# zeromq/libzmq

Hardware: AMD Instinct MI355X
Metric: GiB/s device-resident CURVE encode+decode, 1 KiB-msg batches; msgs/s (higher is better)
Workload: dtype u32; 1 GPU; config2: 65536 x 1024 B frames, 1 CURVE session per GPU, encode+decode round trip; frames_per_gpu=65536, payload_bytes=1024, wire_bytes=1057, sessions=1, parallelism=frame-sharded x1, no collective

## Files before the change

### libzmq_amd/csrc/curve_device.hpp

```cpp
#pragma once

#include <hip/hip_runtime.h>
#include <stdint.h>

namespace zmqg {

__device__ __forceinline__ uint32_t rotl32(uint32_t x, uint32_t n)
{
    return __builtin_rotateleft32(x, n);
}

#define ZMQG_QR(a, b, c, d)        \
    b ^= rotl32(a + d, 7);         \
    c ^= rotl32(b + a, 9);         \
    d ^= rotl32(c + b, 13);        \
    a ^= rotl32(d + c, 18);

#define ZMQG_SALSA20_ROUNDS(x)                                   \
    _Pragma("unroll") for (int rr_ = 0; rr_ < 10; ++rr_)         \
    {                                                            \
        ZMQG_QR(x[0], x[4], x[8], x[12]);                        \
        ZMQG_QR(x[5], x[9], x[13], x[1]);                        \
        ZMQG_QR(x[10], x[14], x[2], x[6]);                       \
        ZMQG_QR(x[15], x[3], x[7], x[11]);                       \
        ZMQG_QR(x[0], x[1], x[2], x[3]);                         \
        ZMQG_QR(x[5], x[6], x[7], x[4]);                         \
        ZMQG_QR(x[10], x[11], x[8], x[9]);                       \
        ZMQG_QR(x[15], x[12], x[13], x[14]);                     \
    }

constexpr uint32_t SIGMA0 = 0x61707865, SIGMA1 = 0x3320646e, SIGMA2 = 0x79622d32, SIGMA3 = 0x6b206574;

__device__ __forceinline__ void salsa20_block(uint32_t out[16], const uint32_t k[8], uint32_t n0, uint32_t n1,
                                              uint32_t ctr_lo, uint32_t ctr_hi)
{
    uint32_t x[16] = {SIGMA0, k[0], k[1], k[2], k[3], SIGMA1, n0, n1,
                      ctr_lo, ctr_hi, SIGMA2, k[4], k[5], k[6], k[7], SIGMA3};
    ZMQG_SALSA20_ROUNDS(x);
    out[0] = x[0] + SIGMA0;
    out[1] = x[1] + k[0];
    out[2] = x[2] + k[1];
    out[3] = x[3] + k[2];
    out[4] = x[4] + k[3];
    out[5] = x[5] + SIGMA1;
    out[6] = x[6] + n0;
    out[7] = x[7] + n1;
    out[8] = x[8] + ctr_lo;
    out[9] = x[9] + ctr_hi;
    out[10] = x[10] + SIGMA2;
    out[11] = x[11] + k[4];
    out[12] = x[12] + k[5];
    out[13] = x[13] + k[6];
    out[14] = x[14] + k[7];
    out[15] = x[15] + SIGMA3;
}

__device__ __forceinline__ void hsalsa20(uint32_t out[8], const uint32_t k[8], const uint32_t in[4])
{
    uint32_t x[16] = {SIGMA0, k[0], k[1], k[2], k[3], SIGMA1, in[0], in[1],
                      in[2], in[3], SIGMA2, k[4], k[5], k[6], k[7], SIGMA3};
    ZMQG_SALSA20_ROUNDS(x);
    out[0] = x[0];
    out[1] = x[5];
    out[2] = x[10];
    out[3] = x[15];
    out[4] = x[6];
    out[5] = x[7];
    out[6] = x[8];
    out[7] = x[9];
}

constexpr uint32_t M26 = 0x3ffffff;

struct fe {
    uint32_t l[5];
};

__device__ __forceinline__ fe fe_zero()
{
    fe z;
    z.l[0] = z.l[1] = z.l[2] = z.l[3] = z.l[4] = 0;
    return z;
}

__device__ __forceinline__ fe fe_one()
{
    fe o = fe_zero();
    o.l[0] = 1;
    return o;
}

__device__ __forceinline__ fe poly_r_from_key(uint32_t k0, uint32_t k1, uint32_t k2, uint32_t k3)
{
    fe r;
    r.l[0] = k0 & 0x3ffffff;
    r.l[1] = __builtin_amdgcn_alignbit(k1, k0, 26) & 0x3ffff03;
    r.l[2] = __builtin_amdgcn_alignbit(k2, k1, 20) & 0x3ffc0ff;
    r.l[3] = __builtin_amdgcn_alignbit(k3, k2, 14) & 0x3f03fff;
    r.l[4] = (k3 >> 8) & 0x00fffff;
    return r;
}

__device__ __forceinline__ void fe_add_block(fe &h, uint32_t m0, uint32_t m1, uint32_t m2, uint32_t m3,
                                             uint32_t hibit)
{
    h.l[0] += m0 & M26;
    h.l[1] += __builtin_amdgcn_alignbit(m1, m0, 26) & M26;
    h.l[2] += __builtin_amdgcn_alignbit(m2, m1, 20) & M26;
    h.l[3] += __builtin_amdgcn_alignbit(m3, m2, 14) & M26;
    h.l[4] += (m3 >> 8) | hibit;
}

__device__ __forceinline__ void fe_add(fe &h, const fe &x)
{
#pragma unroll
    for (int i = 0; i < 5; ++i)
        h.l[i] += x.l[i];
}

__device__ __forceinline__ uint64_t mad64(uint32_t a, uint32_t b, uint64_t c)
{
    return (uint64_t) a * b + c;
}

__device__ __forceinline__ void fe_mul_s(fe &h, const fe &r, const uint32_t s1, const uint32_t s2, const uint32_t s3,
                                         const uint32_t s4)
{
    const uint32_t h0 = h.l[0], h1 = h.l[1], h2 = h.l[2], h3 = h.l[3], h4 = h.l[4];
    uint64_t d0 = mad64(h4, s1, mad64(h3, s2, mad64(h2, s3, mad64(h1, s4, (uint64_t) h0 * r.l[0]))));
    uint64_t d1 = mad64(h4, s2, mad64(h3, s3, mad64(h2, s4, mad64(h1, r.l[0], (uint64_t) h0 * r.l[1]))));
    uint64_t d2 = mad64(h4, s3, mad64(h3, s4, mad64(h2, r.l[0], mad64(h1, r.l[1], (uint64_t) h0 * r.l[2]))));
    uint64_t d3 = mad64(h4, s4, mad64(h3, r.l[0], mad64(h2, r.l[1], mad64(h1, r.l[2], (uint64_t) h0 * r.l[3]))));
    uint64_t d4 = mad64(h4, r.l[0], mad64(h3, r.l[1], mad64(h2, r.l[2], mad64(h1, r.l[3], (uint64_t) h0 * r.l[4]))));
    uint32_t c;
    c = (uint32_t) (d0 >> 26);
    h.l[0] = (uint32_t) d0 & M26;
    d1 += c;
    c = (uint32_t) (d1 >> 26);
    h.l[1] = (uint32_t) d1 & M26;
    d2 += c;
    c = (uint32_t) (d2 >> 26);
    h.l[2] = (uint32_t) d2 & M26;
    d3 += c;
    c = (uint32_t) (d3 >> 26);
    h.l[3] = (uint32_t) d3 & M26;
    d4 += c;
    c = (uint32_t) (d4 >> 26);
    h.l[4] = (uint32_t) d4 & M26;
    h.l[0] += c * 5;
    c = h.l[0] >> 26;
    h.l[0] &= M26;
    h.l[1] += c;
}

__device__ __forceinline__ void fe_mul(fe &h, const fe &r)
{
    fe_mul_s(h, r, r.l[1] * 5, r.l[2] * 5, r.l[3] * 5, r.l[4] * 5);
}

__device__ __forceinline__ fe fe_from_wide(const uint64_t w[5])
{
    uint64_t a0 = w[0], a1 = w[1], a2 = w[2], a3 = w[3], a4 = w[4];
    a1 += a0 >> 26;
    a0 &= M26;
    a2 += a1 >> 26;
    a1 &= M26;
    a3 += a2 >> 26;
    a2 &= M26;
    a4 += a3 >> 26;
    a3 &= M26;
    a0 += (a4 >> 26) * 5;
    a4 &= M26;
    a1 += a0 >> 26;
    a0 &= M26;
    fe h;
    h.l[0] = (uint32_t) a0;
    h.l[1] = (uint32_t) a1;
    h.l[2] = (uint32_t) a2;
    h.l[3] = (uint32_t) a3;
    h.l[4] = (uint32_t) a4;
    return h;
}

__device__ __forceinline__ void poly_finish(fe h, const uint32_t s[4], uint32_t tag[4])
{
    uint32_t h0 = h.l[0], h1 = h.l[1], h2 = h.l[2], h3 = h.l[3], h4 = h.l[4], c;
    c = h1 >> 26;
    h1 &= M26;
    h2 += c;
    c = h2 >> 26;
    h2 &= M26;
    h3 += c;
    c = h3 >> 26;
    h3 &= M26;
    h4 += c;
    c = h4 >> 26;
    h4 &= M26;
    h0 += c * 5;
    c = h0 >> 26;
    h0 &= M26;
    h1 += c;
    uint32_t g0 = h0 + 5;
    c = g0 >> 26;
    g0 &= M26;
    uint32_t g1 = h1 + c;
    c = g1 >> 26;
    g1 &= M26;
    uint32_t g2 = h2 + c;
    c = g2 >> 26;
    g2 &= M26;
    uint32_t g3 = h3 + c;
    c = g3 >> 26;
    g3 &= M26;
    uint32_t g4 = h4 + c - (1u << 26);
    const uint32_t mask = (g4 >> 31) - 1u;
    h0 = (h0 & ~mask) | (g0 & mask);
    h1 = (h1 & ~mask) | (g1 & mask);
    h2 = (h2 & ~mask) | (g2 & mask);
    h3 = (h3 & ~mask) | (g3 & mask);
    h4 = (h4 & ~mask) | (g4 & mask);
    uint64_t f0 = (uint64_t) (h0 | (h1 << 26)) + s[0];
    uint64_t f1 = (uint64_t) ((h1 >> 6) | (h2 << 20)) + s[1] + (f0 >> 32);
    uint64_t f2 = (uint64_t) ((h2 >> 12) | (h3 << 14)) + s[2] + (f1 >> 32);
    uint64_t f3 = (uint64_t) ((h3 >> 18) | (h4 << 8)) + s[3] + (f2 >> 32);
    tag[0] = (uint32_t) f0;
    tag[1] = (uint32_t) f1;
    tag[2] = (uint32_t) f2;
    tag[3] = (uint32_t) f3;
}

__device__ __forceinline__ void poly_absorb64(fe &h, const fe &r, const uint32_t s1, const uint32_t s2,
                                              const uint32_t s3, const uint32_t s4, uint32_t w[16], int nv)
{
    if (nv >= 64) {
#pragma unroll
        for (int q = 0; q < 4; ++q) {
            fe_add_block(h, w[4 * q], w[4 * q + 1], w[4 * q + 2], w[4 * q + 3], 1u << 24);
            fe_mul_s(h, r, s1, s2, s3, s4);
        }
        return;
    }
#pragma unroll
    for (int q = 0; q < 4; ++q) {
        const int bl = nv - 16 * q;
        if (bl <= 0)
            break;
        uint32_t m[4] = {w[4 * q], w[4 * q + 1], w[4 * q + 2], w[4 * q + 3]};
        uint32_t hibit = 1u << 24;
        if (bl < 16) {
            hibit = 0;
            const int wi = bl >> 2, bi = bl & 3;
#pragma unroll
            for (int t = 0; t < 4; ++t)
                if (t == wi)
                    m[t] |= 1u << (8 * bi);
        }
        fe_add_block(h, m[0], m[1], m[2], m[3], hibit);
        fe_mul_s(h, r, s1, s2, s3, s4);
    }
}

struct Poly32 {
    uint32_t h0, h1, h2, h3, h4;
};

struct PolyKey32 {
    uint32_t r0, r1, r2, r3, s1, s2, s3;
};

__device__ __forceinline__ PolyKey32 poly32_key(uint32_t k0, uint32_t k1, uint32_t k2, uint32_t k3)
{
    PolyKey32 k;
    k.r0 = k0 & 0x0fffffffu;
    k.r1 = k1 & 0x0ffffffcu;
    k.r2 = k2 & 0x0ffffffcu;
    k.r3 = k3 & 0x0ffffffcu;
    k.s1 = k.r1 + (k.r1 >> 2);
    k.s2 = k.r2 + (k.r2 >> 2);
    k.s3 = k.r3 + (k.r3 >> 2);
    return k;
}

__device__ __forceinline__ void poly32_block(Poly32 &h, uint32_t m0, uint32_t m1, uint32_t m2, uint32_t m3,
                                             uint32_t hib, const PolyKey32 &k)
{
    unsigned c;
    const uint32_t a0 = __builtin_addc(h.h0, m0, 0u, &c);
    const uint32_t a1 = __builtin_addc(h.h1, m1, c, &c);
    const uint32_t a2 = __builtin_addc(h.h2, m2, c, &c);
    const uint32_t a3 = __builtin_addc(h.h3, m3, c, &c);
    const uint32_t a4 = h.h4 + hib + c;
    const uint64_t d0 = mad64(a3, k.s1, mad64(a2, k.s2, mad64(a1, k.s3, (uint64_t) a0 * k.r0)));
    const uint64_t d1 = mad64(a4, k.s1, mad64(a3, k.s2, mad64(a2, k.s3, mad64(a1, k.r0, (uint64_t) a0 * k.r1))));
    const uint64_t d2 = mad64(a4, k.s2, mad64(a3, k.s3, mad64(a2, k.r0, mad64(a1, k.r1, (uint64_t) a0 * k.r2))));
    const uint64_t d3 = mad64(a4, k.s3, mad64(a3, k.r0, mad64(a2, k.r1, mad64(a1, k.r2, (uint64_t) a0 * k.r3))));
    const uint32_t h0 = (uint32_t) d0;
    const uint32_t h1 = __builtin_addc((uint32_t) d1, (uint32_t) (d0 >> 32), 0u, &c);
    const uint32_t c1 = (uint32_t) (d1 >> 32) + c;
    const uint32_t h2 = __builtin_addc((uint32_t) d2, c1, 0u, &c);
    const uint32_t c2 = (uint32_t) (d2 >> 32) + c;
    const uint32_t h3 = __builtin_addc((uint32_t) d3, c2, 0u, &c);
    const uint32_t h4 = a4 * k.r0 + (uint32_t) (d3 >> 32) + c;
    const uint32_t f = (h4 >> 2) + (h4 & ~3u);
    h.h0 = __builtin_addc(h0, f, 0u, &c);
    h.h1 = __builtin_addc(h1, 0u, c, &c);
    h.h2 = __builtin_addc(h2, 0u, c, &c);
    h.h3 = __builtin_addc(h3, 0u, c, &c);
    h.h4 = (h4 & 3u) + c;
}

__device__ __forceinline__ void poly32_window(Poly32 &h, const PolyKey32 &k, const uint32_t c[16], uint32_t j0,
                                              uint32_t len)
{
#pragma unroll
    for (int j = 0; j < 4; ++j) {
        const int off = 16 * (j - (int) j0);
        if (j >= (int) j0 && off < (int) len) {
            const int nb = (int) len - off;
            uint32_t m0 = c[4 * j], m1 = c[4 * j + 1], m2 = c[4 * j + 2], m3 = c[4 * j + 3], hib = 1u;
            if (nb < 16) {
                hib = 0u;
                const uint32_t pad = 1u << (8 * (nb & 3));
                const int wi = nb >> 2;
                m0 |= wi == 0 ? pad : 0u;
                m1 |= wi == 1 ? pad : 0u;
                m2 |= wi == 2 ? pad : 0u;
                m3 |= wi == 3 ? pad : 0u;
            }
            poly32_block(h, m0, m1, m2, m3, hib, k);
        }
    }
}

__device__ __forceinline__ void poly32_window_full(Poly32 &h, const PolyKey32 &k, const uint32_t c[16])
{
#pragma unroll
    for (int j = 0; j < 4; ++j)
        poly32_block(h, c[4 * j], c[4 * j + 1], c[4 * j + 2], c[4 * j + 3], 1u, k);
}

__device__ __forceinline__ PolyKey32 poly32_key_from_fe(const uint32_t r[5])
{
    return poly32_key(r[0] | (r[1] << 26), (r[1] >> 6) | (r[2] << 20), (r[2] >> 12) | (r[3] << 14),
                      (r[3] >> 18) | (r[4] << 8));
}

__device__ __forceinline__ Poly32 fe_to_poly32(fe x)
{
    uint32_t c;
    c = x.l[0] >> 26;
    x.l[0] &= M26;
    x.l[1] += c;
    c = x.l[1] >> 26;
    x.l[1] &= M26;
    x.l[2] += c;
    c = x.l[2] >> 26;
    x.l[2] &= M26;
    x.l[3] += c;
    c = x.l[3] >> 26;
    x.l[3] &= M26;
    x.l[4] += c;
    Poly32 h;
    h.h0 = x.l[0] | (x.l[1] << 26);
    h.h1 = (x.l[1] >> 6) | (x.l[2] << 20);
    h.h2 = (x.l[2] >> 12) | (x.l[3] << 14);
    h.h3 = (x.l[3] >> 18) | (x.l[4] << 8);
    h.h4 = x.l[4] >> 24;
    return h;
}

__device__ __forceinline__ fe poly32_to_fe(const Poly32 &h)
{
    fe x;
    x.l[0] = h.h0 & M26;
    x.l[1] = ((h.h0 >> 26) | (h.h1 << 6)) & M26;
    x.l[2] = ((h.h1 >> 20) | (h.h2 << 12)) & M26;
    x.l[3] = ((h.h2 >> 14) | (h.h3 << 18)) & M26;
    x.l[4] = (h.h3 >> 8) | (h.h4 << 24);
    return x;
}

__device__ __forceinline__ void poly32_finish(const Poly32 &h, const uint32_t s[4], uint32_t tag[4])
{
    unsigned c;
    const uint32_t g0 = __builtin_addc(h.h0, 5u, 0u, &c);
    const uint32_t g1 = __builtin_addc(h.h1, 0u, c, &c);
    const uint32_t g2 = __builtin_addc(h.h2, 0u, c, &c);
    const uint32_t g3 = __builtin_addc(h.h3, 0u, c, &c);
    const uint32_t g4 = h.h4 + c;
    const uint32_t m = 0u - (g4 >> 2);
    const uint32_t f0 = (g0 & m) | (h.h0 & ~m), f1 = (g1 & m) | (h.h1 & ~m), f2 = (g2 & m) | (h.h2 & ~m),
                   f3 = (g3 & m) | (h.h3 & ~m);
    tag[0] = __builtin_addc(f0, s[0], 0u, &c);
    tag[1] = __builtin_addc(f1, s[1], c, &c);
    tag[2] = __builtin_addc(f2, s[2], c, &c);
    tag[3] = __builtin_addc(f3, s[3], c, &c);
}

__device__ __forceinline__ uint32_t bswap32(uint32_t x)
{
    return __builtin_bswap32(x);
}

__device__ __forceinline__ void mask_tail(uint32_t w[16], int nv)
{
#pragma unroll
    for (int i = 0; i < 16; ++i) {
        const int b = nv - 4 * i;
        const uint32_t m = b >= 4 ? 0xffffffffu : (b <= 0 ? 0u : ((1u << (8 * b)) - 1u));
        w[i] &= m;
    }
}

__device__ __forceinline__ void load_window(const uint8_t *p, int nv, uint32_t w[16])
{
    const uint32_t sh = (uint32_t) ((uintptr_t) p & 3);
    const uint32_t *q = (const uint32_t *) (p - sh);
    uint32_t d[17];
    if (nv >= 64) {
#pragma unroll
        for (int i = 0; i < 16; ++i)
            d[i] = q[i];
        d[16] = sh ? q[16] : 0u;
    } else {
        const int nd = (int) ((sh + (uint32_t) nv + 3) >> 2);
#pragma unroll
        for (int i = 0; i < 17; ++i)
            d[i] = i < nd ? q[i] : 0u;
    }
#pragma unroll
    for (int i = 0; i < 16; ++i)
        w[i] = __builtin_amdgcn_alignbyte(d[i + 1], d[i], sh);
    if (nv < 64)
        mask_tail(w, nv);
}

__device__ __forceinline__ void store_window(uint8_t *p, int nv, const uint32_t w[16])
{
    const uintptr_t a = (uintptr_t) p;
    const uint32_t sh = (uint32_t) (a & 3);
    if (sh == 0 && nv >= 64) {
        typedef unsigned int u32x4_ __attribute__((ext_vector_type(4)));
        typedef __attribute__((address_space(1))) u32x4_ __attribute__((aligned(4))) GU4a4_;
#pragma unroll
        for (int i = 0; i < 4; ++i)
            *(GU4a4_ *) (a + 16u * i) = (u32x4_){w[4 * i], w[4 * i + 1], w[4 * i + 2], w[4 * i + 3]};
        return;
    }
    const uint32_t s = (4u - sh) & 3u;
    (void) a;
    uint32_t e[16];
#pragma unroll
    for (int k = 0; k < 15; ++k)
        e[k] = __builtin_amdgcn_alignbyte(w[k + 1], w[k], s);
    e[15] = __builtin_amdgcn_alignbyte(0u, w[15], s);
    const int lead = (int) s < nv ? (int) s : nv;
#pragma unroll
    for (int b = 0; b < 3; ++b)
        if (b < lead)
            p[b] = (uint8_t) (w[0] >> (8 * b));
    if (nv <= (int) s)
        return;
    const int rem = nv - (int) s;
    const int nd = rem >> 2;
    uint32_t *q = (uint32_t *) (p + s);
#pragma unroll
    for (int k = 0; k < 16; ++k)
        if (k < nd)
            q[k] = e[k];
    const int tb = rem & 3;
    if (tb) {
        uint32_t t = 0;
#pragma unroll
        for (int k = 0; k < 16; ++k)
            if (k == nd)
                t = e[k];
        uint8_t *pt = (uint8_t *) (q + nd);
#pragma unroll
        for (int b = 0; b < 3; ++b)
            if (b < tb)
                pt[b] = (uint8_t) (t >> (8 * b));
    }
}

template <int NV>
__device__ __forceinline__ void store_bytes_c(uint8_t *p, const uint32_t w[16])
{
    static_assert(NV % 4 == 0 && NV >= 8 && NV <= 64, "whole dwords, at most one window");
    typedef __attribute__((address_space(1))) uint8_t GU8_;
    typedef __attribute__((address_space(1))) uint16_t GU16_;
    typedef __attribute__((address_space(1))) uint32_t GU32_;
    typedef unsigned int u32x2_ __attribute__((ext_vector_type(2)));
    typedef unsigned int u32x3_ __attribute__((ext_vector_type(3)));
    typedef __attribute__((address_space(1))) u32x2_ __attribute__((aligned(4))) GU2a4_;
    typedef __attribute__((address_space(1))) u32x3_ __attribute__((aligned(4))) GU3a4_;
    typedef unsigned int u32x4_ __attribute__((ext_vector_type(4)));
    typedef __attribute__((address_space(1))) u32x4_ __attribute__((aligned(4))) GU4a4_;
    const uint64_t a = (uint64_t) (uintptr_t) p;
    const uint32_t sh = (uint32_t) a & 3u, s = (4u - sh) & 3u;
    constexpr int ND = NV / 4;
    uint32_t e[ND];
#pragma unroll
    for (int k = 0; k < ND; ++k)
        e[k] = __builtin_amdgcn_alignbyte(k + 1 < 16 ? w[k + 1] : 0u, w[k], s);
    if (s & 1u)
        *(GU8_ *) (uintptr_t) a = (uint8_t) w[0];
    if (s & 2u)
        *(GU16_ *) (uintptr_t) (a + (s & 1u)) = (uint16_t) (w[0] >> (8u * (s & 1u)));
    const uint64_t q = a + s;
    constexpr int NU = ND - 1;
#pragma unroll
    for (int g = 0; g + 4 <= NU; g += 4)
        *(GU4a4_ *) (uintptr_t) (q + 4u * g) = (u32x4_){e[g], e[g + 1], e[g + 2], e[g + 3]};
    constexpr int G4 = NU / 4 * 4;
    if (NU - G4 == 3)
        *(GU3a4_ *) (uintptr_t) (q + 4u * G4) = (u32x3_){e[G4], e[G4 + 1], e[G4 + 2]};
    else if (NU - G4 == 2)
        *(GU2a4_ *) (uintptr_t) (q + 4u * G4) = (u32x2_){e[G4], e[G4 + 1]};
    else if (NU - G4 == 1)
        *(GU32_ *) (uintptr_t) (q + 4u * G4) = e[G4];
    if (s == 0u)
        *(GU32_ *) (uintptr_t) (q + 4u * NU) = e[NU];
    const uint64_t t = q + 4u * NU;
    if (sh & 2u)
        *(GU16_ *) (uintptr_t) t = (uint16_t) e[NU];
    if (sh & 1u)
        *(GU8_ *) (uintptr_t) (t + (sh & 2u)) = (uint8_t) (e[NU] >> (8u * (sh & 2u)));
}

template <int NV>
__device__ __forceinline__ void load_bytes_c(const uint8_t *p, uint32_t w[NV / 4])
{
    static_assert(NV % 16 == 0 && NV >= 16 && NV <= 48, "whole granules");
    typedef __attribute__((address_space(1))) const uint32_t GCU32_;
    typedef unsigned int u32x4_ __attribute__((ext_vector_type(4)));
    typedef __attribute__((address_space(1))) const u32x4_ __attribute__((aligned(4))) GCU4a4_;
    const uint64_t a = (uint64_t) (uintptr_t) p;
    const uint32_t sh = (uint32_t) a & 3u;
    const uint64_t q = a - sh;
    constexpr int ND = NV / 4;
    uint32_t d[ND + 1];
#pragma unroll
    for (int g = 0; g < ND / 4; ++g) {
        const u32x4_ t = *(GCU4a4_ *) (uintptr_t) (q + 16u * g);
        d[4 * g] = t.x;
        d[4 * g + 1] = t.y;
        d[4 * g + 2] = t.z;
        d[4 * g + 3] = t.w;
    }
    d[ND] = sh ? *(GCU32_ *) (uintptr_t) (q + 4u * ND) : 0u;
#pragma unroll
    for (int k = 0; k < ND; ++k)
        w[k] = __builtin_amdgcn_alignbyte(d[k + 1], d[k], sh);
}

__device__ __forceinline__ void store_tail(uint64_t a, uint32_t nb, const uint32_t o[17])
{
    typedef __attribute__((address_space(1))) uint8_t GU8_;
    typedef __attribute__((address_space(1))) uint16_t GU16_;
    typedef __attribute__((address_space(1))) uint32_t GU32_;
    typedef unsigned int u32x4_ __attribute__((ext_vector_type(4)));
    typedef __attribute__((address_space(1))) u32x4_ __attribute__((aligned(4))) GU4a4_;
    const uint32_t nw = nb >> 2, ng = nw >> 2;
#pragma unroll
    for (uint32_t g = 0; g < 4; ++g)
        if (g < ng)
            *(GU4a4_ *) (uintptr_t) (a + 16u * g) = (u32x4_){o[4 * g], o[4 * g + 1], o[4 * g + 2], o[4 * g + 3]};
    uint32_t r[4];
#pragma unroll
    for (uint32_t k = 0; k < 4; ++k) {
        uint32_t v = 0;
#pragma unroll
        for (uint32_t g = 0; g < 5; ++g)
            if (g == ng && 4 * g + k < 17)
                v = o[4 * g + k];
        r[k] = v;
    }
    const uint64_t b = a + 16u * ng;
    const uint32_t nr = nw - 4u * ng;
#pragma unroll
    for (uint32_t k = 0; k < 3; ++k)
        if (k < nr)
            *(GU32_ *) (uintptr_t) (b + 4u * k) = r[k];
    uint32_t last = r[0];
#pragma unroll
    for (uint32_t k = 1; k < 4; ++k)
        if (k == nr)
            last = r[k];
    const uint32_t tb = nb & 3u;
    const uint64_t c = b + 4u * nr;
    if (tb & 2u)
        *(GU16_ *) (uintptr_t) c = (uint16_t) last;
    if (tb & 1u)
        *(GU8_ *) (uintptr_t) (c + (tb & 2u)) = (uint8_t) (last >> (8u * (tb & 2u)));
}

__device__ __forceinline__ void zero_bytes(uint8_t *p, uint32_t len)
{
    const uint32_t head = (uint32_t) ((16u - ((uintptr_t) p & 15u)) & 15u);
    const uint32_t h = head < len ? head : len;
    for (uint32_t b = 0; b < h; ++b)
        p[b] = 0;
    uint32_t k = h;
    typedef unsigned int z4 __attribute__((ext_vector_type(4)));
    for (; k + 16u <= len; k += 16u)
        *(z4 *) (p + k) = (z4){0u, 0u, 0u, 0u};
    for (; k < len; ++k)
        p[k] = 0;
}

typedef unsigned int u32x4 __attribute__((ext_vector_type(4)));
typedef __attribute__((address_space(1))) uint8_t GU8;
typedef __attribute__((address_space(1))) const u32x4 GCU4;
typedef __attribute__((address_space(1))) u32x4 GU4;
typedef __attribute__((address_space(1))) uint32_t GU32;

template <int N>
__device__ __forceinline__ void select_shift(const uint32_t *v, uint32_t ws, uint32_t *out)
{
    const uint32_t m1 = 0u - (ws & 1u), m2 = 0u - ((ws >> 1) & 1u);
    uint32_t a[N + 2];
#pragma unroll
    for (int i = 0; i < N + 2; ++i)
        a[i] = (v[i + 1] & m1) | (v[i] & ~m1);
#pragma unroll
    for (int i = 0; i < N; ++i)
        out[i] = (a[i + 2] & m2) | (a[i] & ~m2);
}

struct StreamReader {
    const GCU4 *g;
    uint32_t off;
    uint32_t end;
    u32x4 carry;
};

__device__ __forceinline__ void reader_init(StreamReader &r, uint64_t p, uint32_t L)
{
    r.off = (uint32_t) (p & 15);
    r.g = (const GCU4 *) (uintptr_t) (p - r.off);
    r.end = r.off + L;
// ... 155 lines not shown
```

### libzmq_amd/csrc/curve_frames.hpp

```cpp
#pragma once

#ifndef ZMQG_FRAMES_ABLATE
#define ZMQG_FRAMES_ABLATE 0
#endif


#ifndef ZMQG_SEQ_STORE
#define ZMQG_SEQ_STORE 0
#endif

__device__ __forceinline__ void seq_store4(uint64_t a, uint32_t x, uint32_t y, uint32_t z, uint32_t w)
{
    typedef unsigned int v4_ __attribute__((ext_vector_type(4)));
    typedef __attribute__((address_space(1))) v4_ __attribute__((aligned(4))) G4_;
    if (ZMQG_SEQ_STORE == 3)
        asm volatile("global_store_dwordx4 %0, %1, off sc0 sc1\n\ts_nop 1" ::"v"(a), "v"((v4_){x, y, z, w}) : "memory");
    else
        *(G4_ *) (uintptr_t) a = (v4_){x, y, z, w};
}

#ifndef ZMQG_SEQ_COOPST
#define ZMQG_SEQ_COOPST 2
#endif
#ifndef ZMQG_SEQ_SKIP5
// ... 1014 lines not shown
        sh_cs = c0;
    __syncthreads();
    const CallState cs = sh_cs;
    const uint32_t epoch = cs.epoch;
    const uint32_t wg = use_ticket ? cs.ticket : blockIdx.x;
    if (use_ticket)
        fetch(wg);
    const uint64_t nbase = cs.nbase;
    unsigned long long *const list_ctr = zs->list_ctr + (epoch & 1u);
    if (blockIdx.x == 0 && threadIdx.x == 0)
        zs->list_ctr[(epoch & 1u) ^ 1u] = 0;

    if (!DEC) {
        const uint64_t nc = frame_nonce(nonce, ctl, nbase, ii);
        n0 = bswap32((uint32_t) (nc >> 32));
        n1 = bswap32((uint32_t) nc);
    } else {
        if (L_in < 64u)
            mask_tail(x0, (int) L_in);
        const uint32_t b0 = x0[0] & 0xffu;
        if (L_in <= 1u || L_in <= b0)
            status = ZMQG_ERR_MALFORMED_UNSPECIFIED;
        else if (L_in < 8u || x0[0] != 0x53454d07u || x0[1] != 0x45474153u)
            status = ZMQG_ERR_UNEXPECTED_COMMAND;
        else if (L_in < 33u)
            status = ZMQG_ERR_MALFORMED_MESSAGE;
        if (!sid_ok)
            status = ZMQG_ERR_SESSION;
        if (over)
            status = ZMQG_ERR_BOUND;
        n0 = x0[2];
        n1 = x0[3];
        S = status == 0 ? L_in : 0u;
    }
    const bool small = valid && S <= max_stream;
    unsigned long long vn = 0, wexcl = 0, psn = 0, wagg = 0;
    if (DEC) {
        vn = valid && status == 0 ? (((unsigned long long) bswap32(n0) << 32) | bswap32(n1)) : 0ull;
        psn = rp.peer[s];
        if (valid && !lb) {
            rp.vout[i] = vn;
            rp.psnap[i] = psn;
            if (rp.iota)
                rp.iota[i] = i;
        }
        if (lb) {
            const unsigned long long sc = wave_scan_max_u64(vn);
            const unsigned long long up = wave_prev_u64(sc);
            if (lane == 63)
                sh_wmax[threadIdx.x >> 6] = sc;
            __syncthreads();
            const uint32_t wv = threadIdx.x >> 6;
            for (uint32_t k = 0; k < kFramesWaves; ++k) {
                if (k < wv)
                    wexcl = sh_wmax[k] > wexcl ? sh_wmax[k] : wexcl;
                wagg = sh_wmax[k] > wagg ? sh_wmax[k] : wagg;
            }
            if (lane > 0)
                wexcl = up > wexcl ? up : wexcl;
            if (threadIdx.x == 0) {
                if (use_rec) {
                    __hip_atomic_store(rp.lb_rec + 2u * wg, lbrec_pack(epoch, (uint32_t) wagg), __ATOMIC_RELAXED,
                                       __HIP_MEMORY_SCOPE_AGENT);
                    __hip_atomic_store(rp.lb_rec + 2u * wg + 1u, lbrec_pack(epoch, (uint32_t) (wagg >> 32)),
                                       __ATOMIC_RELAXED, __HIP_MEMORY_SCOPE_AGENT);
                } else {
                    lookback_publish(rp.lb_flag + wg, rp.lb_agg + wg, wagg, epoch, 1);
                }
            }
        }
    }
    const bool is_big = valid && !small && S > 0;
    if (!small)
        S = 0;
    const uint32_t nw = (S + 63u) >> 6;
    const uint32_t steps = __builtin_amdgcn_readfirstlane(wave_max_u32(nw));
    __shared__ __attribute__((aligned(16))) uint8_t sq_lds[kFramesWaves * 2 * 64 * kStIn];
    uint8_t *const sq_w = sq_lds + (threadIdx.x >> 6) * 2 * 64 * kStIn;
    const uint32_t sq_off = __builtin_amdgcn_readfirstlane((uint32_t) (uintptr_t) (StLdsVoid *) sq_w);
    const uint32_t sq_va = (uint32_t) A & 15u;
    uint64_t sq_la[5];
    uint32_t sq_rel[5], sq_lim[5];
    {
        const uint64_t Ab = A - sq_va;
        const uint32_t lm = S ? sq_va + S : 0u;
#pragma unroll
        for (uint32_t j = 0; j < 5; ++j) {
            const uint32_t idx = 64u * j + lane, f = idx / 5u, k = idx - 5u * f;
            sq_rel[j] = 16u * k;
            sq_la[j] = shfl_u64(Ab, f) + sq_rel[j];
            sq_lim[j] = (uint32_t) __shfl((int) lm, (int) f);
            const int fva = __shfl((int) sq_va, (int) f);
            if (ZMQG_SEQ_SKIP5 && k == 4u && fva == 0)
                sq_lim[j] = 0;
        }
    }
    auto sq_dma = [&](uint32_t t) {
        const uint32_t b = __builtin_amdgcn_readfirstlane(sq_off + (t & 1u) * 64u * kStIn);
#pragma unroll
        for (uint32_t j = 0; j < 5; ++j)
            if (64u * t + sq_rel[j] < sq_lim[j])
                lds_dma16(sq_la[j] + 64ull * t, b + 1024u * j);
    };
    const uint32_t min_nw = __builtin_amdgcn_readfirstlane(~wave_max_u32(~nw));
    uint64_t sq_m[5];
#pragma unroll
    for (uint32_t j = 0; j < 5; ++j)
        sq_m[j] = __builtin_amdgcn_ballot_w64(sq_lim[j] != 0u);
    auto sq_dma_uni = [&](uint32_t t) {
        const uint32_t b = __builtin_amdgcn_readfirstlane(sq_off + (t & 1u) * 64u * kStIn);
        uint64_t a[5];
#pragma unroll
        for (uint32_t j = 0; j < 5; ++j)
            a[j] = sq_la[j] + 64ull * t;
        unsigned keep;
        uint64_t ex;
        asm volatile("s_mov_b32 %0, m0\n\t"
                     "s_mov_b64 %1, exec\n\t"
                     "s_mov_b32 m0, %7\n\t"
                     "s_mov_b64 exec, %8\n\t"
                     "global_load_lds_dwordx4 %2, off\n\t"
                     "s_add_u32 m0, m0, 0x400\n\t"
                     "s_mov_b64 exec, %9\n\t"
                     "global_load_lds_dwordx4 %3, off\n\t"
                     "s_add_u32 m0, m0, 0x400\n\t"
                     "s_mov_b64 exec, %10\n\t"
                     "global_load_lds_dwordx4 %4, off\n\t"
                     "s_add_u32 m0, m0, 0x400\n\t"
                     "s_mov_b64 exec, %11\n\t"
                     "global_load_lds_dwordx4 %5, off\n\t"
                     "s_add_u32 m0, m0, 0x400\n\t"
                     "s_mov_b64 exec, %12\n\t"
                     "global_load_lds_dwordx4 %6, off\n\t"
                     "s_mov_b64 exec, %1\n\t"
                     "s_mov_b32 m0, %0"
                     : "=&s"(keep), "=&s"(ex)
                     : "v"(a[0]), "v"(a[1]), "v"(a[2]), "v"(a[3]), "v"(a[4]), "s"(b), "s"(sq_m[0]), "s"(sq_m[1]),
                       "s"(sq_m[2]), "s"(sq_m[3]), "s"(sq_m[4])
                     : "memory", "scc");
    };
    if (steps > 1u && !(ZMQG_FRAMES_ABLATE & 16))
        sq_dma(1u);

    const bool al64 = ZMQG_SEQ_AL64 && DEC && __builtin_amdgcn_ballot_w64(((uint32_t) (uintptr_t) dst & 63u) != 0u) == 0;
    uint32_t yp[16];
    bool cs_pend = false;
    constexpr uint32_t kStgPlane = 64u * 16u + 16u;
    __shared__ __attribute__((aligned(16))) uint8_t sq_stg[ZMQG_SEQ_COOPST && SO ? kFramesWaves * 4 * kStgPlane : 16];
    uint8_t *const stg = sq_stg + (ZMQG_SEQ_COOPST && SO ? (threadIdx.x >> 6) * 4u * kStgPlane : 0u);
    auto stg_put = [&](uint32_t k) { return stg + kStgPlane * k + 16u * lane; };
    auto stg_get = [&](uint32_t j) { return stg + kStgPlane * (lane & 3u) + 16u * (16u * j + (lane >> 2)); };
    uint64_t cs_dst[4];
    uint32_t cs_nw[4];
    const bool coop = ZMQG_SEQ_COOPST && SO && (DEC ? al64 : true);
    if (coop) {
        const uint64_t cbase = DEC ? (uint64_t) (uintptr_t) dst : B - (((uint32_t) B & 3u) ? ((uint32_t) B & 3u) : 4u);
#pragma unroll
        for (uint32_t j = 0; j < 4; ++j) {
            const uint32_t f = 16u * j + (lane >> 2);
            cs_dst[j] = shfl_u64(cbase, f) + 16u * (lane & 3u);
            cs_nw[j] = (uint32_t) __shfl((int) nw, (int) f);
        }
    }
    uint32_t ct0[8];

    SEQ_STAMP(1u);
    PolyKey32 pk;
    Poly32 h = {0, 0, 0, 0, 0};
    uint32_t spad[4], wtag[4] = {0, 0, 0, 0}, fl = 0;
    uint32_t cp[16];
    uint32_t cp_j0 = 2, cp_len = 0;
    uint32_t ycarry;
    {
        uint32_t ks[16];
        salsa20_block(ks, key, n0, n1, 0, 0);
        pk = poly32_key(ks[0], ks[1], ks[2], ks[3]);
#pragma unroll
        for (int k = 0; k < 4; ++k)
            spad[k] = ks[4 + k];
        uint32_t x[16];
        if (DEC) {
#pragma unroll
            for (int k = 0; k < 16; ++k)
                x[k] = x0[k];
#pragma unroll
            for (int k = 0; k < 4; ++k)
                wtag[k] = x[4 + k];
        } else {
            uint32_t pt[8];
            switch (hl) {
            case 1: shift_in<1>(x0, pt); break;
            case 2: shift_in<2>(x0, pt); break;
            case 8: shift_in<8>(x0, pt); break;
            default: shift_in<11>(x0, pt); break;
            }
            pt[0] |= hw[0];
            pt[1] |= hw[1];
            pt[2] |= hw[2];
#pragma unroll
            for (int k = 0; k < 8; ++k) {
                x[k] = 0;
                x[8 + k] = pt[k];
            }
        }
        uint32_t y[16];
#pragma unroll
        for (int k = 0; k < 16; ++k)
            y[k] = x[k] ^ ks[k];
        if (!DEC && S < 64u)
            mask_tail(y, (int) S);
#pragma unroll
        for (int k = 0; k < 16; ++k)
            cp[k] = DEC ? x[k] : y[k];
        cp_len = (S < 64u ? S : 64u) - 32u;
        ycarry = y[15];
#pragma unroll
        for (int k = 0; k < 16; ++k)
            yp[k] = y[k];
        if (nw > 0) {
            if (DEC) {
                fl = y[8] & 3u;
                uint32_t pay[16];
#pragma unroll
                for (int k = 0; k < 7; ++k)
                    pay[k] = __builtin_amdgcn_alignbyte(y[9 + k], y[8 + k], 1);
                pay[7] = __builtin_amdgcn_alignbyte(0u, y[15], 1);
#pragma unroll
                for (int k = 8; k < 16; ++k)
                    pay[k] = 0;
                if (!al64 || nw == 1u)
                    store_window(dst, (int) (S < 64u ? S : 64u) - 33, pay);
            } else {
#pragma unroll
                for (int k = 0; k < 8; ++k)
                    ct0[k] = y[8 + k];
                if (S < 64u) {
                    uint32_t o[16];
                    o[0] = 0x53454d07u;
                    o[1] = 0x45474153u;
                    o[2] = n0;
                    o[3] = n1;
#pragma unroll
                    for (int k = 4; k < 16; ++k)
                        o[k] = 0;
                    store_bytes_c<16>(dst, o);
                    uint32_t ct[16];
#pragma unroll
                    for (int k = 0; k < 16; ++k)
                        ct[k] = k < 8 ? y[8 + k] : 0u;
                    store_window(dst + 32, (int) S - 32, ct);
                }
            }
        }
    }
    SEQ_STAMP(2u);
    call_state_count(zs);

    auto step = [&](auto uni, uint32_t t) {
        constexpr bool UNI = decltype(uni)::value;
        SEQ_STAMP(3u + t);
        const bool act = UNI || t < nw;
        const bool had = ZMQG_SEQ_COOPST && coop && cs_pend;
        u32x4 cg[4];
        if (had) {
            __builtin_amdgcn_fence(__ATOMIC_SEQ_CST, "wavefront");
#pragma unroll
            for (uint32_t j = 0; j < 4; ++j)
                cg[j] = *(const u32x4 *) stg_get(j);
        }
        uint32_t ks[16];
        if (ZMQG_FRAMES_ABLATE & 32) {
#pragma unroll
            for (int k = 0; k < 16; ++k)
                ks[k] = key[k & 7] ^ (t * 0x9e3779b9u + k);
        } else {
            salsa20_block(ks, key, n0, n1, t, 0);
        }
#pragma unroll
        for (int k = 0; k < 16; ++k)
            asm volatile("" : "+v"(ks[k]));
        SEQ_STAMP(24u + t);
        asm volatile("s_waitcnt vmcnt(0)" ::: "memory");
        __builtin_amdgcn_fence(__ATOMIC_SEQ_CST, "wavefront");
        uint32_t x[16];
        {
            const uint8_t *const p = sq_w + (t & 1u) * 64u * kStIn + kStIn * lane + sq_va;
#pragma unroll
            for (uint32_t q = 0; q < 4; ++q) {
                const u32x4 u = *(const u32x4_u1 *) (p + 16u * q);
                x[4 * q] = u.x;
                x[4 * q + 1] = u.y;
                x[4 * q + 2] = u.z;
                x[4 * q + 3] = u.w;
            }
        }
        asm volatile("" : "+v"(h.h0), "+v"(h.h1), "+v"(h.h2), "+v"(h.h3), "+v"(h.h4));
        const bool pv = UNI || t - 1u < nw;
        const bool full = UNI || (pv && cp_j0 == 0u && cp_len == 64u);
        {
            Poly32 hf = h;
            if (ZMQG_FRAMES_ABLATE & 64)
                hf.h0 ^= cp[0] ^ cp[5] ^ cp[11];
            else
                poly32_window_full(hf, pk, cp);
            h.h0 = full ? hf.h0 : h.h0;
            h.h1 = full ? hf.h1 : h.h1;
            h.h2 = full ? hf.h2 : h.h2;
            h.h3 = full ? hf.h3 : h.h3;
            h.h4 = full ? hf.h4 : h.h4;
        }
        asm volatile(""
                     : "+v"(h.h0), "+v"(h.h1), "+v"(h.h2), "+v"(h.h3), "+v"(h.h4), "+v"(ks[0]), "+v"(ks[1]), "+v"(ks[2]),
                       "+v"(ks[3]), "+v"(ks[4]), "+v"(ks[5]), "+v"(ks[6]), "+v"(ks[7]), "+v"(ks[8]), "+v"(ks[9]),
                       "+v"(ks[10]), "+v"(ks[11]), "+v"(ks[12]), "+v"(ks[13]), "+v"(ks[14]), "+v"(ks[15]));
        if (!UNI && !(ZMQG_FRAMES_ABLATE & 64) && __builtin_amdgcn_ballot_w64(pv && !full) != 0) {
            if (pv && !full)
                poly32_window(h, pk, cp, cp_j0, cp_len);
        }
        if (t < 8u)
            SEQ_STAMP(44u + t);
        const bool tail = !UNI && act && S < 64u * t + 64u;
        if (!UNI && DEC && __builtin_amdgcn_ballot_w64(tail) != 0) {
            if (tail)
                mask_tail(x, (int) (S - 64u * t));
        }
        uint32_t y[16];
#pragma unroll
        for (int k = 0; k < 16; ++k)
            y[k] = x[k] ^ ks[k];
        if (!UNI && !DEC && __builtin_amdgcn_ballot_w64(tail) != 0) {
            if (tail)
                mask_tail(y, (int) (S - 64u * t));
        }
#pragma unroll
        for (int k = 0; k < 16; ++k)
            cp[k] = DEC ? x[k] : y[k];
        cp_j0 = 0;
        cp_len = UNI ? 64u : act ? (S - 64u * t < 64u ? S - 64u * t : 64u) : 0u;
        if (!(ZMQG_FRAMES_ABLATE & 16)) {
            if (UNI)
                sq_dma_uni(t + 1u);
            else if (t + 1u < steps)
                sq_dma(t + 1u);
        }
        if (t < 8u)
            SEQ_STAMP(52u + t);
        const bool lastw = !UNI && act && t + 1u == nw;
        const bool no_last = UNI || __builtin_amdgcn_ballot_w64(lastw) == 0;
        if (ZMQG_FRAMES_ABLATE & 8) {
            if (act && y[3] == 0x12345678u && y[7] == ycarry)
                *(GU32 *) (uintptr_t) B = y[0];
        } else if (DEC && al64) {
            uint32_t o[16];
#pragma unroll
            for (int k = 0; k < 7; ++k)
                o[k] = __builtin_amdgcn_alignbyte(yp[9 + k], yp[8 + k], 1);
            o[7] = __builtin_amdgcn_alignbyte(y[0], yp[15], 1);
#pragma unroll
            for (int k = 8; k < 16; ++k)
                o[k] = __builtin_amdgcn_alignbyte(y[k - 7], y[k - 8], 1);
            uint8_t *const cdst = dst + 64u * (t - 1u);
            if (had) {
#pragma unroll
                for (uint32_t j = 0; j < 4; ++j)
                    if (UNI || t - 1u < cs_nw[j])
                        seq_store4(cs_dst[j] + 64ull * (t - 2u), cg[j].x, cg[j].y, cg[j].z, cg[j].w);
                cs_pend = false;
            }
            if (ZMQG_SEQ_COOPST && coop && no_last) {
                __builtin_amdgcn_fence(__ATOMIC_SEQ_CST, "wavefront");
#pragma unroll
                for (int k = 0; k < 4; ++k)
                    *(u32x4 *) stg_put(k) = (u32x4){o[4 * k], o[4 * k + 1], o[4 * k + 2], o[4 * k + 3]};
                cs_pend = true;
            } else if (no_last) {
                if (act) {
#pragma unroll
                    for (int k = 0; k < 4; ++k)
                        seq_store4((uint64_t) (uintptr_t) cdst + 16u * k, o[4 * k], o[4 * k + 1], o[4 * k + 2],
                                   o[4 * k + 3]);
                }
            } else {
                const uint32_t P = S - 33u;
                if (act) {
                    const uint32_t r = P - 64u * (t - 1u);
                    const uint32_t o17[17] = {o[0], o[1], o[2],  o[3],  o[4],  o[5],  o[6],  o[7], o[8],
                                              o[9], o[10], o[11], o[12], o[13], o[14], o[15], 0u};
                    store_tail((uint64_t) (uintptr_t) cdst, r < 64u ? r : 64u, o17);
                }
                if (lastw && P > 64u * t) {
                    uint32_t o2[17];
#pragma unroll
                    for (int k = 0; k < 7; ++k)
                        o2[k] = __builtin_amdgcn_alignbyte(y[9 + k], y[8 + k], 1);
                    o2[7] = __builtin_amdgcn_alignbyte(0u, y[15], 1);
#pragma unroll
                    for (int k = 8; k < 17; ++k)
                        o2[k] = 0;
                    store_tail((uint64_t) (uintptr_t) (cdst + 64), P - 64u * t, o2);
                }
            }
#pragma unroll
            for (int k = 0; k < 16; ++k)
                yp[k] = y[k];
        } else {
            if constexpr (!DEC) {
                if (had) {
#pragma unroll
                    for (uint32_t j = 0; j < 4; ++j)
                        if (UNI || t - 1u < cs_nw[j])
                            seq_store4(cs_dst[j] + 64ull * (t - 1u), cg[j].x, cg[j].y, cg[j].z, cg[j].w);
                    cs_pend = false;
                }
            }
            if (!DEC && ZMQG_SEQ_COOPST && coop && no_last) {
                const uint32_t u = (uint32_t) B & 3u, sh = u ? 4u - u : 0u;
                uint32_t o[16];
                o[0] = __builtin_amdgcn_alignbyte(y[0], ycarry, sh);
#pragma unroll
                for (int k = 1; k < 16; ++k)
                    o[k] = __builtin_amdgcn_alignbyte(y[k], y[k - 1], sh);
                __builtin_amdgcn_fence(__ATOMIC_SEQ_CST, "wavefront");
#pragma unroll
                for (int k = 0; k < 4; ++k)
                    *(u32x4 *) stg_put(k) = (u32x4){o[4 * k], o[4 * k + 1], o[4 * k + 2], o[4 * k + 3]};
                cs_pend = true;
            } else if (UNI) {
                frame_store(B, t, 0xffffffffu, y, ycarry, false);
            } else if (act) {
                frame_store(B, t, S, y, ycarry, lastw);
            }
        }
        ycarry = y[15];
        if (t < 8u)
            SEQ_STAMP(36u + t);
    };
    if (steps > 1u) {
#pragma unroll 1
        for (uint32_t t = 1; t < steps; ++t) {
            if (ZMQG_SEQ_UNI && t >= 2u && t + 2u < min_nw)
                step(std::true_type{}, t);
            else
                step(std::false_type{}, t);
        }
    }
    SEQ_STAMP(60u);
    unsigned long long rl[4] = {0, 0, 0, 0}, rh[4] = {0, 0, 0, 0};
    if (use_rec) {
#pragma unroll
        for (uint32_t q = 0; q < 4; ++q) {
            const int k = (int) wg - 1 - (int) (lane + 64u * q);
            const unsigned long long *const r = rp.lb_rec + 2u * (uint32_t) (k >= 0 ? k : 0);
            rl[q] = __hip_atomic_load(r, __ATOMIC_RELAXED, __HIP_MEMORY_SCOPE_AGENT);
            rh[q] = __hip_atomic_load(r + 1, __ATOMIC_RELAXED, __HIP_MEMORY_SCOPE_AGENT);
        }
        asm volatile("" : "+v"(h.h0), "+v"(h.h1), "+v"(h.h2), "+v"(h.h3), "+v"(h.h4)::"memory");
    }
    if (steps > 0 && nw == steps)
        poly32_window(h, pk, cp, cp_j0, cp_len);
    uint32_t tag[4];
    poly32_finish(h, spad, tag);

    unsigned long long excl = 0;
    if (use_rec) {
        unsigned long long P = 0;
#pragma unroll
        for (uint32_t q = 0; q < 4; ++q) {
            const int k = (int) wg - 1 - (int) (lane + 64u * q);
            if (k >= 0) {
                const unsigned long long *const r = rp.lb_rec + 2u * (uint32_t) k;
                while (!lbrec_valid(rl[q], epoch)) {
                    __builtin_amdgcn_s_sleep(1);
                    rl[q] = __hip_atomic_load(r, __ATOMIC_RELAXED, __HIP_MEMORY_SCOPE_AGENT);
                }
                while (!lbrec_valid(rh[q], epoch)) {
                    __builtin_amdgcn_s_sleep(1);
                    rh[q] = __hip_atomic_load(r + 1, __ATOMIC_RELAXED, __HIP_MEMORY_SCOPE_AGENT);
                }
                P = max_u64(P, lbrec_value(rl[q], rh[q]));
            }
        }
        P = wave_max_u64(P);
        if (threadIdx.x == 0 && wg + 1 == gridDim.x) {
            const unsigned long long inc = P > wagg ? P : wagg;
            *rp.peer = inc > psn ? inc : psn;
            if (rp.smax)
                *rp.smax = inc;
        }
        excl = P > wexcl ? P : wexcl;
        if (excl < psn)
            excl = psn;
    } else if (lb) {
        const unsigned long long P = lookback_excl(wg, epoch, rp.lb_flag, rp.lb_agg, rp.lb_inc);
        if (threadIdx.x == 0) {
            const unsigned long long inc = P > wagg ? P : wagg;
            if (gridDim.x > kFramesBS)
                lookback_publish(rp.lb_flag + wg, rp.lb_inc + wg, inc, epoch, 2);
            if (wg + 1 == gridDim.x) {
                *rp.peer = inc > psn ? inc : psn;
                if (rp.smax)
                    *rp.smax = inc;
            }
        }
        excl = P > wexcl ? P : wexcl;
        if (excl < psn)
            excl = psn;
    }
    if (is_big && !ctl.no_body) {
        if (lb) {
            rp.excl[i] = excl;
            rp.psnap[i] = psn;
        }
        big(i, list_ctr, nbase);
    }
    call_state_end<DEC>(zs, ctl, cs, n);
    frame_result_copy<DEC>(big);
    SEQ_STAMP(61u);
#if ZMQG_SEQ_STAMPS
    if (rp.clk && (threadIdx.x & 63u) == 0)
        rp.clk[64ull * (blockIdx.x * kFramesWaves + (threadIdx.x >> 6)) + 62u] =
            ((unsigned long long) __builtin_amdgcn_s_getreg((31 << 11) | 20) << 32) |
            __builtin_amdgcn_s_getreg((31 << 11) | 4);
#endif
    if (!DEC && valid && ctl.enc_status)
        ctl.enc_status[i] = !sid_ok ? ZMQG_ERR_SESSION : over ? ZMQG_ERR_BOUND : 0;
    if (!valid || !small)
        return;
    if (S == 0) {
        if (DEC)
            fail_unprocessed(status, L_in, dst, flags_out + i, status_out + i, zs, ctl);
        return;
    }
    if (!DEC) {
        if (S >= 64u) {
            const uint32_t o[16] = {0x53454d07u, 0x45474153u, n0,     n1,     tag[0], tag[1], tag[2], tag[3],
                                    ct0[0],      ct0[1],      ct0[2], ct0[3], ct0[4], ct0[5], ct0[6], ct0[7]};
            store_bytes_c<64>(dst, o);
        } else {
            const uint32_t o[16] = {tag[0], tag[1], tag[2], tag[3]};
            store_bytes_c<16>(dst + 16, o);
        }
    } else {
        if (lb && !(vn > excl))
            status = ZMQG_ERR_INVALID_SEQUENCE;
        else if ((tag[0] ^ wtag[0]) | (tag[1] ^ wtag[1]) | (tag[2] ^ wtag[2]) | (tag[3] ^ wtag[3]))
            status = ZMQG_ERR_CRYPTOGRAPHIC;
        status_out[i] = status;
        flags_out[i] = status == 0 ? (uint8_t) (fl | frame_zbits<DEC>(big, i)) : 0;
        if (status != 0) {
            asm volatile("s_waitcnt vmcnt(0)" ::: "memory");
            zero_bytes(dst, S - 33u);
        }
    }
}

template <bool DEC, class BigOp, bool SO = false>
__global__ __launch_bounds__(kFramesBS) ZMQG_SEQ_ATTR void k_frames_seq(ZMQG_FRAMES_PARAMS)
{
    frames_seq_impl<DEC, BigOp, SO>(ZMQG_FRAMES_ARGS);
}

template <bool DEC, int GT, class BigOp>
__global__ __launch_bounds__(kFramesBS) ZMQG_SEQ_ATTR void k_frames_split(ZMQG_FRAMES_PARAMS)
{
    if (blockIdx.x < ctl.split_wg)
        frames_seq_impl<DEC, BigOp>(ZMQG_FRAMES_ARGS);
    else
        frames_g_impl<DEC, GT, BigOp>(ZMQG_FRAMES_ARGS);
}

}
```

Baseline: 621.7 GiB/s.

## Fold Poly1305 carry chain into MAD ops and extend uniform step path

Rewrites the Poly1305 block update so the next message block's limbs and carry propagation are folded into 64-bit multiply-add chains, using SGPR constants 1. This replaces the addc carry chain and the separate final normalization between consecutive blocks in a full window. It also lets step t=1 take the uniform fast path, where only the last two blocks of that window are hashed (from2). This assumes the first 32 bytes of window 1 are not part of the MAC. The looser limb normalization between blocks and the from2 assumption both carry correctness risk.

```diff
diff --git a/libzmq_amd/csrc/curve_device.hpp b/libzmq_amd/csrc/curve_device.hpp
--- a/libzmq_amd/csrc/curve_device.hpp
+++ b/libzmq_amd/csrc/curve_device.hpp
@@ -281,32 +281,73 @@
     return k;
 }
 
+__device__ __forceinline__ uint32_t poly32_one()
+{
+    uint32_t one;
+    asm("s_mov_b32 %0, 1" : "=s"(one));
+    return one;
+}
+
+__device__ __forceinline__ uint32_t poly32_uno()
+{
+    uint32_t uno;
+    asm("s_movk_i32 %0, 1" : "=s"(uno));
+    return uno;
+}
+
+template <bool NEXT>
+__device__ __forceinline__ Poly32 poly32_mul_add(const Poly32 &a, const PolyKey32 &k, uint32_t n0, uint32_t n1,
+                                                 uint32_t n2, uint32_t n3, uint32_t nhib)
+{
+    const uint32_t one = poly32_one(), uno = poly32_uno();
+    uint64_t d0 = mad64(a.h3, k.s1, mad64(a.h2, k.s2, mad64(a.h1, k.s3, (uint64_t) a.h0 * k.r0)));
+    const uint64_t d1 =
+        mad64(a.h4, k.s1, mad64(a.h3, k.s2, mad64(a.h2, k.s3, mad64(a.h1, k.r0, (uint64_t) a.h0 * k.r1))));
+    const uint64_t d2 =
+        mad64(a.h4, k.s2, mad64(a.h3, k.s3, mad64(a.h2, k.r0, mad64(a.h1, k.r1, (uint64_t) a.h0 * k.r2))));
+    const uint64_t d3 =
+        mad64(a.h4, k.s3, mad64(a.h3, k.r0, mad64(a.h2, k.r1, mad64(a.h1, k.r2, (uint64_t) a.h0 * k.r3))));
+    const uint32_t d3h = (uint32_t) (d3 >> 32);
+    const uint32_t g = a.h4 * k.r0 + d3h;
+    d0 = mad64(g >> 2, 5u, d0);
+    const uint32_t w = (g & 3u) - d3h;
+    if (NEXT)
+        d0 = mad64(n0, uno, d0);
+    uint64_t t1 = mad64((uint32_t) (d0 >> 32), one, d1);
+    if (NEXT)
+        t1 = mad64(n1, uno, t1);
+    uint64_t t2 = mad64((uint32_t) (t1 >> 32), one, d2);
+    if (NEXT)
+        t2 = mad64(n2, uno, t2);
+    uint64_t t3 = mad64((uint32_t) (t2 >> 32), one, d3);
+    if (NEXT)
+        t3 = mad64(n3, uno, t3);
+    Poly32 o;
+    o.h0 = (uint32_t) d0;
+    o.h1 = (uint32_t) t1;
+    o.h2 = (uint32_t) t2;
+    o.h3 = (uint32_t) t3;
+    o.h4 = (uint32_t) (t3 >> 32) + w + (NEXT ? nhib : 0u);
+    return o;
+}
+
+__device__ __forceinline__ Poly32 poly32_add(const Poly32 &h, uint32_t m0, uint32_t m1, uint32_t m2, uint32_t m3,
+                                             uint32_t hib)
+{
+    unsigned c;
+    Poly32 a;
+    a.h0 = __builtin_addc(h.h0, m0, 0u, &c);
+    a.h1 = __builtin_addc(h.h1, m1, c, &c);
+    a.h2 = __builtin_addc(h.h2, m2, c, &c);
+    a.h3 = __builtin_addc(h.h3, m3, c, &c);
+    a.h4 = h.h4 + hib + c;
+    return a;
+}
+
 __device__ __forceinline__ void poly32_block(Poly32 &h, uint32_t m0, uint32_t m1, uint32_t m2, uint32_t m3,
                                              uint32_t hib, const PolyKey32 &k)
 {
-    unsigned c;
-    const uint32_t a0 = __builtin_addc(h.h0, m0, 0u, &c);
-    const uint32_t a1 = __builtin_addc(h.h1, m1, c, &c);
-    const uint32_t a2 = __builtin_addc(h.h2, m2, c, &c);
-    const uint32_t a3 = __builtin_addc(h.h3, m3, c, &c);
-    const uint32_t a4 = h.h4 + hib + c;
-    const uint64_t d0 = mad64(a3, k.s1, mad64(a2, k.s2, mad64(a1, k.s3, (uint64_t) a0 * k.r0)));
-    const uint64_t d1 = mad64(a4, k.s1, mad64(a3, k.s2, mad64(a2, k.s3, mad64(a1, k.r0, (uint64_t) a0 * k.r1))));
-    const uint64_t d2 = mad64(a4, k.s2, mad64(a3, k.s3, mad64(a2, k.r0, mad64(a1, k.r1, (uint64_t) a0 * k.r2))));
-    const uint64_t d3 = mad64(a4, k.s3, mad64(a3, k.r0, mad64(a2, k.r1, mad64(a1, k.r2, (uint64_t) a0 * k.r3))));
-    const uint32_t h0 = (uint32_t) d0;
-    const uint32_t h1 = __builtin_addc((uint32_t) d1, (uint32_t) (d0 >> 32), 0u, &c);
-    const uint32_t c1 = (uint32_t) (d1 >> 32) + c;
-    const uint32_t h2 = __builtin_addc((uint32_t) d2, c1, 0u, &c);
-    const uint32_t c2 = (uint32_t) (d2 >> 32) + c;
-    const uint32_t h3 = __builtin_addc((uint32_t) d3, c2, 0u, &c);
-    const uint32_t h4 = a4 * k.r0 + (uint32_t) (d3 >> 32) + c;
-    const uint32_t f = (h4 >> 2) + (h4 & ~3u);
-    h.h0 = __builtin_addc(h0, f, 0u, &c);
-    h.h1 = __builtin_addc(h1, 0u, c, &c);
-    h.h2 = __builtin_addc(h2, 0u, c, &c);
-    h.h3 = __builtin_addc(h3, 0u, c, &c);
-    h.h4 = (h4 & 3u) + c;
+    h = poly32_mul_add<false>(poly32_add(h, m0, m1, m2, m3, hib), k, 0u, 0u, 0u, 0u, 0u);
 }
 
 __device__ __forceinline__ void poly32_window(Poly32 &h, const PolyKey32 &k, const uint32_t c[16], uint32_t j0,
@@ -332,11 +373,19 @@
     }
 }
 
-__device__ __forceinline__ void poly32_window_full(Poly32 &h, const PolyKey32 &k, const uint32_t c[16])
-{
-#pragma unroll
-    for (int j = 0; j < 4; ++j)
-        poly32_block(h, c[4 * j], c[4 * j + 1], c[4 * j + 2], c[4 * j + 3], 1u, k);
+__device__ __forceinline__ void poly32_window_full(Poly32 &h, const PolyKey32 &k, const uint32_t c[16],
+                                                   bool from2 = false)
+{
+    Poly32 a;
+    if (from2) {
+        a = poly32_add(h, c[8], c[9], c[10], c[11], 1u);
+    } else {
+        a = poly32_add(h, c[0], c[1], c[2], c[3], 1u);
+        a = poly32_mul_add<true>(a, k, c[4], c[5], c[6], c[7], 1u);
+        a = poly32_mul_add<true>(a, k, c[8], c[9], c[10], c[11], 1u);
+    }
+    a = poly32_mul_add<true>(a, k, c[12], c[13], c[14], c[15], 1u);
+    h = poly32_mul_add<false>(a, k, 0u, 0u, 0u, 0u, 0u);
 }
 
 __device__ __forceinline__ PolyKey32 poly32_key_from_fe(const uint32_t r[5])
diff --git a/libzmq_amd/csrc/curve_frames.hpp b/libzmq_amd/csrc/curve_frames.hpp
--- a/libzmq_amd/csrc/curve_frames.hpp
+++ b/libzmq_amd/csrc/curve_frames.hpp
@@ -1340,7 +1340,7 @@
             if (ZMQG_FRAMES_ABLATE & 64)
                 hf.h0 ^= cp[0] ^ cp[5] ^ cp[11];
             else
-                poly32_window_full(hf, pk, cp);
+                poly32_window_full(hf, pk, cp, UNI && __builtin_amdgcn_readfirstlane(t) == 1u);
             h.h0 = full ? hf.h0 : h.h0;
             h.h1 = full ? hf.h1 : h.h1;
             h.h2 = full ? hf.h2 : h.h2;
@@ -1476,7 +1476,7 @@
     if (steps > 1u) {
 #pragma unroll 1
         for (uint32_t t = 1; t < steps; ++t) {
-            if (ZMQG_SEQ_UNI && t >= 2u && t + 2u < min_nw)
+            if (ZMQG_SEQ_UNI && t + 2u < min_nw)
                 step(std::true_type{}, t);
             else
                 step(std::false_type{}, t);
```

Result: faster. 648.3 GiB/s (median of 6 runs) (+4.3%).
